# rezashkv/diffusion_pruning

Hardware: AMD Instinct MI355X
Metric: denoise-steps/s (SD-2.1 U-Net forward, 512x512, bs=4 per GPU, 50% channel mask) (higher is better)
Workload: dtype bf16

## Files before the change

### diffusion_pruning_amd/csrc/conv_gemm.hip

```cpp
#define APTP_CG_MAIN 1
#include "conv_gemm_core.h"

using namespace aptp_cg;

namespace {

template <typename T> struct Elem;
template <> struct Elem<__bf16> { static constexpr int EPC = 8, KS = 64; };
template <> struct Elem<float> { static constexpr int EPC = 4, KS = 32; };

template <int BM, int BN, int WM, int WN, typename T = __bf16>
__global__ __launch_bounds__(256) void conv_gemm_kernel(const KParams p) {
  static_assert(WM * WN == 4, "4 waves per workgroup");
  constexpr int EPC = Elem<T>::EPC, KS = Elem<T>::KS, ES = (int)sizeof(T);
  constexpr bool F32 = sizeof(T) == 4;
  constexpr int WTM = BM / WM, WTN = BN / WN;
  constexpr int MF = WTM / 16, NF = WTN / 16;
  constexpr int A_PASS = BM / 32, B_PASS = BN / 32;
  static_assert(BM % 32 == 0 && BN % 32 == 0 && WTM % 16 == 0 && WTN % 16 == 0, "tile shape");

  __shared__ __attribute__((aligned(16))) T smem[2 * (BM + BN) * KS];
  T* As = smem;
  T* Bs = smem + 2 * BM * KS;

// ... 1250 lines not shown
    mp = (M + kTiles[t].bm - 1) / kTiles[t].bm * kTiles[t].bm;
    np = ((int64_t)p->N + kTiles[t].bn - 1) / kTiles[t].bn * kTiles[t].bn;
  }
  return (int64_t)p->split_k * mp * np * (int64_t)sizeof(float);
}

extern "C" int aptp_conv_gemm_tiles(const AptpConvGemmParams* p) {
  if (!p) return 0;
  const int64_t M = (int64_t)p->B * p->Hout * p->Wout;
  const int t = pick_tile(p, (int)M);
  if (t <= 0 || t >= kNumTiles) return 0;
  return (int)(((M + kTiles[t].bm - 1) / kTiles[t].bm) * ((p->N + kTiles[t].bn - 1) / kTiles[t].bn));
}

extern "C" int aptp_conv_gemm_colstat_rows(const AptpConvGemmParams* p) {
  if (!p) return 0;
  const int t = pick_tile(p, p->B * p->Hout * p->Wout);
  if (t <= 0 || t >= kNumTiles) return 0;
  return kTiles[t].bm / (kTiles[t].nw / kTiles[t].wn);
}

extern "C" int aptp_conv_gemm_rowstat_slots(const AptpConvGemmParams* p) {
  if (!p) return 0;
  const int t = pick_tile(p, p->B * p->Hout * p->Wout);
  if (t <= 0 || t >= kNumTiles) return 0;
  return ((p->N + kTiles[t].bn - 1) / kTiles[t].bn) * kTiles[t].wn;
}

extern "C" int aptp_conv_gemm_suggest_split_k(const AptpConvGemmParams* p) {
  if (!p) return 1;
  const int M = p->B * p->Hout * p->Wout;
  const int t = pick_tile(p, M);
  const int64_t blocks = (int64_t)((M + kTiles[t].bm - 1) / kTiles[t].bm) * ((p->N + kTiles[t].bn - 1) / kTiles[t].bn);
  const int nK = p->KH * p->KW * (p->cin_pad / BK);
  if (blocks >= 256) return 1;
  int s = (int)((512 + blocks - 1) / blocks);
  const int max_s = nK / 8 > 0 ? nK / 8 : 1;
  if (s > max_s) s = max_s;
  if (s > 32) s = 32;
  return s < 1 ? 1 : s;
}

extern "C" int aptp_conv_gemm(const AptpConvGemmParams* p, aptp_stream_t stream) {
  KParams k;
  const int rc = fill_kparams(p, k);
  if (rc != APTP_OK) return rc;
  if (k.split_k > 1) APTP_CHECK(k.ws != nullptr && ((uintptr_t)k.ws % 16) == 0, "conv_gemm: split_k > 1 needs a 16B-aligned workspace");
  if (k.split_k == 1) k.counters = nullptr;
  k.gn_gamma = p->gn_gamma; k.gn_beta = p->gn_beta; k.gn_groups = p->gn_groups; k.gn_C = p->gn_C; k.gn_silu = p->gn_silu; k.gn_eps = p->gn_eps;
  if (k.gn_gamma) {
    APTP_CHECK(k.gn_beta && k.split_k > 1 && !k.counters && !k.out_f32 && k.act == APTP_ACT_NONE && !k.colgate && !k.corr && !k.residual && !k.depth
               && !k.rstat_out && !k.cstat_out && !k.ln_stats, "conv_gemm: gn_gamma needs a plain bf16 convolution split along K with a reduce launch");
    APTP_CHECK(k.gn_groups > 0 && k.gn_C > 0 && k.gn_C <= k.N && k.gn_C % k.gn_groups == 0 && k.gn_C % 8 == 0 && (k.gn_C / k.gn_groups) % 4 == 0
               && (int64_t)k.HW * (k.gn_C / k.gn_groups) <= 4LL * GN_RED_QPT * GN_RED_NT && k.ldy % 4 == 0,
               "conv_gemm: gn_gamma geometry (C=%d groups=%d HW=%d)", k.gn_C, k.gn_groups, k.HW);
  }
  hipStream_t s = (hipStream_t)stream;
  int t = pick_tile(p, k.M);
  if (t < 0 || t >= kNumTiles) { aptp_set_error("conv_gemm: unknown tile %d", t); return APTP_EINVAL; }
  if (k.io_f32 && t >= APTP_TILE_DMA_128x128) {
    aptp_set_error("conv_gemm: io_f32 (fp32 parity path) runs on the register-staged tiles 1..6 only (got tile %d)", t);
    return APTP_EINVAL;
  }
  if (t >= APTP_TILE_DMA_128x128 && !is_sk_tile(t) && (p->cin_pad * 2 > 8064 || (p->x2 && p->cin2_pad * 2 > 8064))) {
    aptp_set_error("conv_gemm: LDS-DMA tiles need Cin <= 4032 (got cin_pad %d)", p->cin_pad);
    return APTP_EINVAL;
  }
  if (k.rstat_out) {
    const int slots = ((k.N + kTiles[t].bn - 1) / kTiles[t].bn) * kTiles[t].wn;
    if ((k.split_k != 1 && !k.counters) || k.rstat_slots != slots) {
      aptp_set_error("conv_gemm: rowstat_out needs split_k == 1 (or the in-kernel reduction) and rowstat_slots == aptp_conv_gemm_rowstat_slots() (%d), got split_k %d, slots %d",
                     slots, k.split_k, k.rstat_slots);
      return APTP_EINVAL;
    }
  }
  if (k.cstat_out) {
    const int wtm = kTiles[t].bm / (kTiles[t].nw / kTiles[t].wn), wtn = kTiles[t].bn / kTiles[t].wn;
    if (!k.epi16 || k.act == APTP_ACT_GEGLU || (k.split_k != 1 && !k.counters) || k.HW % wtm != 0 || wtn < 32 ||
        k.cstat_ld < k.Nout || ((uintptr_t)k.cstat_out % 8) != 0) {
      aptp_set_error("conv_gemm: colstat_out needs the coalesced bf16 epilogue, no GEGLU, split_k == 1 (or the in-kernel reduction), "
                     "Hout*Wout %% %d == 0 (aptp_conv_gemm_colstat_rows) and colstat_ld >= N", wtm);
      return APTP_EINVAL;
    }
  }
  if (k.act == APTP_ACT_GEGLU && (kTiles[t].bn == 160)) {
    aptp_set_error("conv_gemm: GEGLU cannot use a 160-wide tile");
    return APTP_EINVAL;
  }
  {
    const int tiles_m = (k.M + kTiles[t].bm - 1) / kTiles[t].bm, tiles_n = (k.N + kTiles[t].bn - 1) / kTiles[t].bn;
    APTP_CHECK((int64_t)tiles_m * tiles_n * k.split_k < (1ll << 31) && (int64_t)k.nK * (k.split_k + 1) < (1ll << 31), "conv_gemm: grid too large");
    k.fd_hw = make_fastdiv(k.HW); k.fd_wout = make_fastdiv(k.Wout);
    k.fd_tm = make_fastdiv(tiles_m); k.fd_tn = make_fastdiv(tiles_n); k.fd_sk = make_fastdiv(k.split_k);
    k.fd_perm = make_fastdiv(tiles_n * k.split_k); k.fd_tmn = make_fastdiv(tiles_m * tiles_n);
  }
  static const bool lin_on = !(getenv("APTP_LIN") && getenv("APTP_LIN")[0] == '0');
  if (lin_on && p->epilogue != 2 && aptp_lin_eligible(k, t)) {
    const int rc2 = aptp_launch_lin(k, t, s);
    if (rc2 != APTP_OK) return rc2;
    APTP_LAUNCH_CHECK();
    return APTP_OK;
  }
  switch (t) {
    case APTP_TILE_128x128: launch_tile<128, 128>(k, s); break;
    case APTP_TILE_128x160: launch_tile<128, 160>(k, s); break;
    case APTP_TILE_64x128: launch_tile<64, 128>(k, s); break;
    case APTP_TILE_64x160: launch_tile<64, 160>(k, s); break;
    case APTP_TILE_128x64: launch_tile<128, 64>(k, s); break;
    case APTP_TILE_64x64: launch_tile<64, 64>(k, s); break;
    case APTP_TILE_DMA_128x128: launch_tile_dma<128, 128, 2>(k, s); break;
    case APTP_TILE_DMA_128x160: launch_tile_dma<128, 160, 2>(k, s); break;
    case APTP_TILE_DMA_64x128: launch_tile_dma<64, 128, 2>(k, s); break;
    case APTP_TILE_DMA_64x160: launch_tile_dma<64, 160, 2>(k, s); break;
    case APTP_TILE_DMA_128x64: launch_tile_dma<128, 64, 2>(k, s); break;
    case APTP_TILE_DMA_64x64: launch_tile_dma<64, 64, 2>(k, s); break;
    case APTP_TILE_DMA3_128x128: launch_tile_dma<128, 128, 3>(k, s); break;
    case APTP_TILE_DMA3_128x160: launch_tile_dma<128, 160, 3>(k, s); break;
    case APTP_TILE_DMA3_64x128: launch_tile_dma<64, 128, 3>(k, s); break;
    case APTP_TILE_DMA3_64x160: launch_tile_dma<64, 160, 3>(k, s); break;
    case APTP_TILE_DMA3_128x64: launch_tile_dma<128, 64, 3>(k, s); break;
    case APTP_TILE_DMA3_64x64: launch_tile_dma<64, 64, 3>(k, s); break;
    case APTP_TILE_DMA8_128x160: launch_tile_dma8<128, 160, 4, 2>(k, s); break;
    case APTP_TILE_DMA8_256x160: launch_tile_dma8<256, 160, 4, 2>(k, s); break;
    case APTP_TILE_DMA8_128x128: launch_tile_dma8<128, 128, 2, 4>(k, s); break;
    case APTP_TILE_DMA8_256x128: launch_tile_dma8<256, 128, 4, 2>(k, s); break;
    case APTP_TILE_DMA4_64x160: launch_tile_dma<64, 160, 4>(k, s); break;
    case APTP_TILE_DMA4_64x128: launch_tile_dma<64, 128, 4>(k, s); break;
    case APTP_TILE_DMA4_64x64: launch_tile_dma<64, 64, 4>(k, s); break;
    case APTP_TILE_DMA4_128x64: launch_tile_dma<128, 64, 4>(k, s); break;
    case APTP_TILE_DMA4_128x128: launch_tile_dma<128, 128, 4>(k, s); break;
    case APTP_TILE_DMA8R3_128x160: launch_tile_dma8<128, 160, 4, 2, 3>(k, s); break;
    case APTP_TILE_DMA8R4_128x160: launch_tile_dma8<128, 160, 4, 2, 4>(k, s); break;
    case APTP_TILE_DMA8R3_128x128: launch_tile_dma8<128, 128, 2, 4, 3>(k, s); break;
    case APTP_TILE_DMA8R4_128x128: launch_tile_dma8<128, 128, 2, 4, 4>(k, s); break;
    case APTP_TILE_DMA8R3_256x128: launch_tile_dma8<256, 128, 4, 2, 3>(k, s); break;
    case APTP_TILE_PP3_128x160: launch_tile_pp<128, 160, 4, 2, 3>(k, s); break;
    case APTP_TILE_PP4_128x160: launch_tile_pp<128, 160, 4, 2, 4>(k, s); break;
    case APTP_TILE_PP3_128x128: launch_tile_pp<128, 128, 2, 4, 3>(k, s); break;
    case APTP_TILE_PP4_128x128: launch_tile_pp<128, 128, 2, 4, 4>(k, s); break;
    case APTP_TILE_PP4_64x160: launch_tile_pp<64, 160, 4, 2, 4>(k, s); break;
    case APTP_TILE_PP4_64x128: launch_tile_pp<64, 128, 2, 4, 4>(k, s); break;
    case APTP_TILE_PP5_64x160: launch_tile_pp<64, 160, 4, 2, 5>(k, s); break;
    case APTP_TILE_PP4_128x64: launch_tile_pp<128, 64, 4, 2, 4>(k, s); break;
    case APTP_TILE_PP3_256x128: launch_tile_pp<256, 128, 4, 2, 3>(k, s); break;
    case APTP_TILE_PP3_128x256: launch_tile_pp<128, 256, 2, 4, 3>(k, s); break;
    case APTP_TILE_DMA6_64x64: launch_tile_dma<64, 64, 6>(k, s); break;
    case APTP_TILE_DMA8S_64x64: launch_tile_dma<64, 64, 8>(k, s); break;
    case APTP_TILE_DMA6_64x128: launch_tile_dma<64, 128, 6>(k, s); break;
    case APTP_TILE_DMA6_128x64: launch_tile_dma<128, 64, 6>(k, s); break;
    case APTP_TILE_KU2S4_64x64: launch_tile_ku2<64, 64, 2, 2, 4>(k, s); break;
    case APTP_TILE_KU2S6_64x64: launch_tile_ku2<64, 64, 2, 2, 6>(k, s); break;
    case APTP_TILE_KU2S4_64x128: launch_tile_ku2<64, 128, 2, 2, 4>(k, s); break;
    case APTP_TILE_KU2S6_64x128: launch_tile_ku2<64, 128, 2, 2, 6>(k, s); break;
    case APTP_TILE_KU2S4_128x64: launch_tile_ku2<128, 64, 2, 2, 4>(k, s); break;
    case APTP_TILE_KU2S4_128x128: launch_tile_ku2<128, 128, 2, 2, 4>(k, s); break;
    case APTP_TILE_KU2S4_64x160: launch_tile_ku2<64, 160, 2, 2, 4>(k, s); break;
    case APTP_TILE_KU2S4_128x160: launch_tile_ku2<128, 160, 4, 2, 4>(k, s); break;
    case APTP_TILE_KU2S4_128x128W8: launch_tile_ku2<128, 128, 2, 4, 4>(k, s); break;
    case APTP_TILE_KS2S3_64x64: launch_tile_ks2<64, 64, 3>(k, s); break;
    case APTP_TILE_KS2S4_64x64: launch_tile_ks2<64, 64, 4>(k, s); break;
    case APTP_TILE_KS2S3_64x128: launch_tile_ks2<64, 128, 3>(k, s); break;
    case APTP_TILE_KS2S4_64x128: launch_tile_ks2<64, 128, 4>(k, s); break;
    case APTP_TILE_KS2S3_128x64: launch_tile_ks2<128, 64, 3>(k, s); break;
    case APTP_TILE_KS2S3_128x128: launch_tile_ks2<128, 128, 3>(k, s); break;
    case APTP_TILE_SK_256x160: case APTP_TILE_SK_256x128: case APTP_TILE_SK_128x256:
    case APTP_TILE_SKL_256x160: case APTP_TILE_SKL_256x128: case APTP_TILE_SKL_128x256:
    case APTP_TILE_SK_128x160: case APTP_TILE_SKL_128x160: case APTP_TILE_SK_128x128: case APTP_TILE_SKL_128x128: {
      if (k.split_k > 1 && !k.counters) { aptp_set_error("conv_gemm: the stream-K tiles combine in-kernel: split_k > 1 needs tile_counters"); return APTP_EINVAL; }
      const int rc2 = aptp_launch_sk(k, t, s);
      if (rc2 != APTP_OK) return rc2;
      break;
    }
    case APTP_TILE_HALO_128x160:
    case APTP_TILE_HALO_128x128: {
      const int W = p->Wout;
      if (!(p->KH == 3 && p->KW == 3 && p->stride == 1 && p->pad == 1 && p->ups == 0 && !p->x2 && W > 0 && 128 % W == 0 &&
            (p->Hout * W) % 128 == 0 && (128 / W + 2) * (W + 2) <= 264)) {
        aptp_set_error("conv_gemm: the halo tiles need a 3x3 / stride-1 / pad-1 convolution without x2 whose width divides 128 (16, 32 or 64)");
        return APTP_EINVAL;
      }
      const int tiles = ((k.M + 127) / 128) * ((k.N + kTiles[t].bn - 1) / kTiles[t].bn);
      if (t == APTP_TILE_HALO_128x160) hipLaunchKernelGGL((conv3x3_halo_kernel<160, 4>), dim3(tiles * k.split_k), dim3(512), 0, s, k);
      else hipLaunchKernelGGL((conv3x3_halo_kernel<128, 4>), dim3(tiles * k.split_k), dim3(512), 0, s, k);
      break;
    }
// ... 16 lines not shown
```

### diffusion_pruning_amd/csrc/conv_gemm_core.h

```cpp
#pragma once
#include "aptp_common.h"
#if defined(APTP_STAMPS) && defined(APTP_CG_MAIN)
__device__ unsigned long long g_stamps[4096 * 4];
__device__ unsigned long long g_phase[4096 * 8];
#define APTP_PHASE(i) do { st_phase[i] = __builtin_readcyclecounter() - st_entry; } while (0)
__device__ unsigned long long g_epi[4096 * 8];
#define APTP_EPI(k) do { if ((threadIdx.x & 63) == 0) g_epi[((blockIdx.x * 8 + (threadIdx.x >> 6)) & 4095) * 8 + (k)] = __builtin_readcyclecounter(); } while (0)
#define APTP_STAMP(i) do { asm volatile("s_waitcnt lgkmcnt(0)" ::: "memory"); const unsigned long long t_ = __builtin_readcyclecounter(); \
    if ((i) > 0) st_acc[(i) - 1] += t_ - st_prev; st_prev = t_; } while (0)
#else
#define APTP_STAMP(i) do { } while (0)
#define APTP_PHASE(i) do { } while (0)
#define APTP_EPI(k) do { } while (0)
#endif
#ifndef APTP_ABLATE
#define APTP_ABLATE 0
#endif

namespace aptp_cg {


constexpr int BK = 64;
typedef __attribute__((ext_vector_type(4))) unsigned int u32x4;

// ... 273 lines not shown
    lna[i] += __shfl_xor(lna[i], 16); lna2[i] += __shfl_xor(lna2[i], 16);
    lna[i] += __shfl_xor(lna[i], 32); lna2[i] += __shfl_xor(lna2[i], 32);
    RowCtx rc;
    ln_finish(p, lna[i], lna2[i], rc);
    ln_mean[i] = rc.mean; ln_rstd[i] = rc.rstd;
  }
}

template <int MF, int NF, int WTM, int WTN, int WN>
__device__ __forceinline__ void tile_epilogue(const KParams& p, f32x4 (&acc)[MF][NF], int m0, int n0, int tn, int wm, int wn, int lane,
                                              const float (&ln_mean)[MF], const float (&ln_rstd)[MF]) {
  const int frow = lane & 15, fq = lane >> 4;
#pragma unroll
  for (int i = 0; i < MF; ++i) {
    const int m = m0 + wm * WTM + i * 16 + frow;
    if (m >= p.M) continue;
    RowCtx rc;
    row_info(p, m, rc);
    rc.mean = ln_mean[i]; rc.rstd = ln_rstd[i];
    float st[2] = {0.f, 0.f};
    if (p.act == APTP_ACT_GEGLU) {
      if constexpr (NF % 2 == 0) {
#pragma unroll
        for (int j = 0; j < NF; j += 2) {
          const int n = n0 + wn * WTN + j * 16 + fq * 4;
          if (n >= p.N) continue;
          float h[4] = {acc[i][j][0], acc[i][j][1], acc[i][j][2], acc[i][j][3]};
          float g[4] = {acc[i][j + 1][0], acc[i][j + 1][1], acc[i][j + 1][2], acc[i][j + 1][3]};
          epilogue_quad<true>(p, m, rc, n, h, g, st);
        }
      }
    } else {
#pragma unroll
      for (int j = 0; j < NF; ++j) {
        const int n = n0 + wn * WTN + j * 16 + fq * 4;
        if (n >= p.N) continue;
        float h[4] = {acc[i][j][0], acc[i][j][1], acc[i][j][2], acc[i][j][3]};
        epilogue_quad<false>(p, m, rc, n, h, h, st);
      }
    }
    if (p.rstat_out) {
      st[0] += __shfl_xor(st[0], 16); st[1] += __shfl_xor(st[1], 16);
      st[0] += __shfl_xor(st[0], 32); st[1] += __shfl_xor(st[1], 32);
      if (fq == 0) {
        float2 o; o.x = st[0]; o.y = st[1];
        const int slot = tn * WN + wn;
        reinterpret_cast<float2*>(p.rstat_out)[((int64_t)(slot >> 1) * p.M + m) * 2 + (slot & 1)] = o;
      }
    }
  }
}

constexpr float USTAT_SUM_SCALE = 1048576.0f;
constexpr float USTAT_SQ_SCALE = 4096.0f;
template <int WL>
__device__ __forceinline__ void emit_unit_stats(const KParams& p, const float (&tot)[2][(WL + 63) / 64], float* buf, int lane, int cw0,
                                                int row0) {
  __builtin_amdgcn_fence(__ATOMIC_ACQ_REL, "wavefront");
  __builtin_amdgcn_wave_barrier();
#pragma unroll
  for (int q = 0; q < (WL + 63) / 64; ++q) {
    const int t = lane + 64 * q;
    if (t < WL) { buf[t] = tot[0][q]; buf[WL + t] = tot[1][q]; }
  }
  __builtin_amdgcn_fence(__ATOMIC_ACQ_REL, "wavefront");
  __builtin_amdgcn_wave_barrier();
  const int cend = cw0 + WL < p.Nout ? cw0 + WL : p.Nout;
  if (cw0 >= cend || row0 >= p.M) return;
  const int unit = p.ustat_unit;
  const int u0 = cw0 / unit, u1 = (cend - 1) / unit;
  const int u = u0 + lane;
  if (u > u1) return;
  const int lo = (u * unit > cw0 ? u * unit : cw0) - cw0;
  const int hi = ((u + 1) * unit < cend ? (u + 1) * unit : cend) - cw0;
  float s = 0.f, s2 = 0.f;
  for (int c = lo; c < hi; ++c) { s += buf[c]; s2 += buf[WL + c]; }
  const int b = p.fd_hw.div(row0);
  const int rep = (int)blockIdx.x & (p.ustat_nrep - 1);
  unsigned long long* dst = reinterpret_cast<unsigned long long*>(p.ustat_out) + (((int64_t)rep * p.B + b) * p.ustat_units + u) * 2;
  __hip_atomic_fetch_add(dst, (unsigned long long)__float2ll_rn(s * USTAT_SUM_SCALE), __ATOMIC_RELAXED, __HIP_MEMORY_SCOPE_AGENT);
  __hip_atomic_fetch_add(dst + 1, (unsigned long long)__float2ll_rn(s2 * USTAT_SQ_SCALE), __ATOMIC_RELAXED, __HIP_MEMORY_SCOPE_AGENT);
}

template <bool GEGLU, int MF, int NF, int WTM, int WTN, int WN>
__device__ __forceinline__ void tile_epilogue_lds(const KParams& p, f32x4 (&acc)[MF][NF], int m0, int n0, int tn, int wm, int wn,
                                                  int lane, const float (&ln_mean)[MF], const float (&ln_rstd)[MF], float* buf) {
  constexpr int WL = GEGLU ? WTN / 2 : WTN;
  constexpr int PITCH = WL + 4;
  constexpr int LPR = WL / 8;
  constexpr int RPP = 64 / LPR;
  constexpr int NPASS = (16 + RPP - 1) / RPP;
  constexpr bool POW2 = (LPR & (LPR - 1)) == 0;
  const int frow = lane & 15, fq = lane >> 4;
  const int lrow = lane / LPR, lc8 = lane - lrow * LPR;
  const int c0 = (GEGLU ? ((n0 + wn * WTN) >> 1) : (n0 + wn * WTN)) + lc8 * 8;
  const bool lane_on = lrow < RPP && c0 < p.Nout;
  __bf16* const yb = reinterpret_cast<__bf16*>(p.y);
  float cs[8], cs2[8];
#pragma unroll
  for (int e = 0; e < 8; ++e) { cs[e] = 0.f; cs2[e] = 0.f; }
#pragma unroll
  for (int i = 0; i < MF; ++i) {
    const int mbase = m0 + wm * WTM + i * 16;
    u32x4 rres[NPASS], rdin[NPASS];
#pragma unroll
    for (int ps = 0; ps < NPASS; ++ps) {
      const int r = ps * RPP + lrow, m2 = mbase + r;
      const bool on = lane_on && r < 16 && m2 < p.M;
      rres[ps] = (u32x4){0u, 0u, 0u, 0u}; rdin[ps] = (u32x4){0u, 0u, 0u, 0u};
      if (on && p.residual && !(APTP_ABLATE & 64)) rres[ps] = *reinterpret_cast<const u32x4*>(p.residual + (int64_t)m2 * p.ldres + c0);
      if (on && p.depth && !(APTP_ABLATE & 64)) rdin[ps] = *reinterpret_cast<const u32x4*>(p.depth_in + (int64_t)m2 * p.lddin + c0);
    }
    {
      const int m = mbase + frow;
      RowCtx rc;
      row_info(p, m < p.M ? m : p.M - 1, rc);
      rc.mean = ln_mean[i]; rc.rstd = ln_rstd[i];
      if constexpr (GEGLU) {
        if constexpr (NF % 2 == 0) {
#pragma unroll
          for (int j = 0; j < NF; j += 2) {
            const int n = n0 + wn * WTN + j * 16 + fq * 4;
            float h[4] = {acc[i][j][0], acc[i][j][1], acc[i][j][2], acc[i][j][3]};
            float g[4] = {acc[i][j + 1][0], acc[i][j + 1][1], acc[i][j + 1][2], acc[i][j + 1][3]};
            float v[4] = {0.f, 0.f, 0.f, 0.f};
            if (n < p.N) {
              ColVecs cv;
              load_colvecs<true>(p, n, cv);
              epilogue_pre<true>(p, rc, n, cv, h, g, v);
            }
            *reinterpret_cast<float4*>(buf + frow * PITCH + (j / 2) * 16 + fq * 4) = make_float4(v[0], v[1], v[2], v[3]);
          }
        }
      } else {
#pragma unroll
        for (int j = 0; j < NF; ++j) {
          const int n = n0 + wn * WTN + j * 16 + fq * 4;
          float h[4] = {acc[i][j][0], acc[i][j][1], acc[i][j][2], acc[i][j][3]};
          float v[4] = {0.f, 0.f, 0.f, 0.f};
          if (n < p.N) {
            ColVecs cv;
            load_colvecs<false>(p, n, cv);
            epilogue_pre<false>(p, rc, n, cv, h, h, v);
          }
          *reinterpret_cast<float4*>(buf + frow * PITCH + j * 16 + fq * 4) = make_float4(v[0], v[1], v[2], v[3]);
        }
      }
    }
    __builtin_amdgcn_fence(__ATOMIC_ACQ_REL, "wavefront");
    __builtin_amdgcn_wave_barrier();
    if (i == 0) APTP_EPI(2);
#pragma unroll
    for (int ps = 0; ps < NPASS; ++ps) {
      const int r = ps * RPP + lrow, m2 = mbase + r;
      const bool on = lane_on && r < 16 && m2 < p.M;
      float v[8];
      {
        const int rr = r < 16 ? r : 15;
        const float4 a = *reinterpret_cast<const float4*>(buf + rr * PITCH + lc8 * 8);
        const float4 b4 = *reinterpret_cast<const float4*>(buf + rr * PITCH + lc8 * 8 + 4);
        v[0] = a.x; v[1] = a.y; v[2] = a.z; v[3] = a.w; v[4] = b4.x; v[5] = b4.y; v[6] = b4.z; v[7] = b4.w;
      }
      if (p.residual && !(APTP_ABLATE & 64)) {
        float f[8];
        union { u32x4 v; uint4 s; } cv; cv.v = rres[ps];
        unpack_bf16x8(cv.s, f);
#pragma unroll
        for (int e = 0; e < 8; ++e) v[e] += f[e];
      }
      if (p.depth && !(APTP_ABLATE & 64)) {
        const float d = p.depth[p.fd_hw.div(m2 < p.M ? m2 : p.M - 1) % p.depth_B];
        float f[8];
        union { u32x4 v; uint4 s; } cv; cv.v = rdin[ps];
        unpack_bf16x8(cv.s, f);
#pragma unroll
        for (int e = 0; e < 8; ++e) v[e] = (1.0f - d) * f[e] + d * v[e];
      }
      const uint4 o = pack_bf16x8(v);
#if APTP_ABLATE & 32
      asm volatile("" :: "v"(o.x), "v"(o.y), "v"(o.z), "v"(o.w));
#else
      if (on) *reinterpret_cast<uint4*>(yb + (int64_t)m2 * p.ldy + c0) = o;
#endif
      if constexpr (!GEGLU) {
        if (p.cstat_out && on) {
          float f[8];
          unpack_bf16x8(o, f);
#pragma unroll
          for (int e = 0; e < 8; ++e) { cs[e] += f[e]; cs2[e] += f[e] * f[e]; }
        }
      }
      if constexpr (POW2) {
        if (p.rstat_out) {
          float f[8], s0 = 0.f, s1 = 0.f;
          unpack_bf16x8(o, f);
          if (c0 < p.Nout) {
#pragma unroll
            for (int e = 0; e < 8; ++e) { s0 += f[e]; s1 += f[e] * f[e]; }
          }
#pragma unroll
          for (int off = 1; off < LPR; off <<= 1) { s0 += __shfl_xor(s0, off); s1 += __shfl_xor(s1, off); }
          if (lrow < RPP && r < 16 && m2 < p.M && lc8 == 0) {
            float2 q; q.x = s0; q.y = s1;
            const int slot = tn * WN + wn;
            reinterpret_cast<float2*>(p.rstat_out)[((int64_t)(slot >> 1) * p.M + m2) * 2 + (slot & 1)] = q;
          }
        }
      }
    }
    if (i == 0) APTP_EPI(3);
  }
  APTP_EPI(4);
  if constexpr (!GEGLU && WL >= 32) {
    if (p.cstat_out) {
      static_assert(RPP * WL <= 16 * PITCH, "column-statistics staging");
      float tot[2][(WL + 63) / 64];
#pragma unroll
      for (int ph = 0; ph < 2; ++ph) {
        if (lrow < RPP) {
          float* dst = buf + lrow * WL + lc8 * 8;
          if (ph == 0) {
            *reinterpret_cast<float4*>(dst) = make_float4(cs[0], cs[1], cs[2], cs[3]);
            *reinterpret_cast<float4*>(dst + 4) = make_float4(cs[4], cs[5], cs[6], cs[7]);
          } else {
            *reinterpret_cast<float4*>(dst) = make_float4(cs2[0], cs2[1], cs2[2], cs2[3]);
            *reinterpret_cast<float4*>(dst + 4) = make_float4(cs2[4], cs2[5], cs2[6], cs2[7]);
          }
        }
        __builtin_amdgcn_fence(__ATOMIC_ACQ_REL, "wavefront");
        __builtin_amdgcn_wave_barrier();
#pragma unroll
        for (int q = 0; q < (WL + 63) / 64; ++q) {
          const int t = lane + 64 * q;
          float a = 0.f;
          if (t < WL) {
#pragma unroll
            for (int r = 0; r < RPP; ++r) a += buf[r * WL + t];
          }
          tot[ph][q] = a;
        }
        __builtin_amdgcn_fence(__ATOMIC_ACQ_REL, "wavefront");
        __builtin_amdgcn_wave_barrier();
      }
      const int cw0 = n0 + wn * WTN;
      float2* dstg = reinterpret_cast<float2*>(p.cstat_out) + (int64_t)(m0 / WTM + wm) * p.cstat_ld;
#pragma unroll
      for (int q = 0; q < (WL + 63) / 64; ++q) {
        const int t = lane + 64 * q;
        if (t < WL && cw0 + t < p.Nout) dstg[cw0 + t] = make_float2(tot[0][q], tot[1][q]);
      }
      if (p.ustat_out) emit_unit_stats<WL>(p, tot, buf, lane, cw0, m0 + wm * WTM);
    }
  }
}

template <int NT, int MF, int NF>
__device__ __forceinline__ bool splitk_combine(const KParams& p, f32x4 (&acc)[MF][NF], int tile, int kz, int tid, int* lds_word) {
  constexpr int PER = MF * NF;
  float4* const slab = reinterpret_cast<float4*>(p.ws) + (int64_t)tile * p.split_k * (PER * NT);
  float4* const mine = slab + (int64_t)kz * (PER * NT);
  {
    const __amdgpu_buffer_rsrc_t srsrc = __builtin_amdgcn_make_buffer_rsrc(mine, 0, PER * NT * 16, 0x00020000);
#pragma unroll
    for (int i = 0; i < MF; ++i)
#pragma unroll
      for (int j = 0; j < NF; ++j) {
        __builtin_amdgcn_raw_buffer_store_b128(__builtin_bit_cast(u32x4, acc[i][j]), srsrc, ((i * NF + j) * NT + tid) * 16, 0, 16);
      }
  }
  asm volatile("s_waitcnt vmcnt(0)" ::: "memory");
  __syncthreads();
  if (tid == 0) *lds_word = __hip_atomic_fetch_add(p.counters + tile, 1, __ATOMIC_RELAXED, __HIP_MEMORY_SCOPE_AGENT);
  __syncthreads();
  const int ticket = *reinterpret_cast<volatile int*>(lds_word);
  if (ticket != p.split_k - 1) return false;
  if (tid == 0) {
    __hip_atomic_store(p.counters + tile, 0, __ATOMIC_RELAXED, __HIP_MEMORY_SCOPE_AGENT);
    __builtin_amdgcn_fence(__ATOMIC_ACQUIRE, "agent");
    asm volatile("s_waitcnt vmcnt(0)" ::: "memory");
  }
  __syncthreads();
#pragma unroll
  for (int i = 0; i < MF; ++i)
#pragma unroll
    for (int j = 0; j < NF; ++j) acc[i][j] = (f32x4){0.f, 0.f, 0.f, 0.f};
  for (int z = 0; z < p.split_k; ++z) {
    const float4* src = slab + (int64_t)z * (PER * NT);
    float4 t[MF][NF];
#pragma unroll
    for (int i = 0; i < MF; ++i)
#pragma unroll
      for (int j = 0; j < NF; ++j) t[i][j] = src[(i * NF + j) * NT + tid];
#pragma unroll
    for (int i = 0; i < MF; ++i)
#pragma unroll
      for (int j = 0; j < NF; ++j) {
        acc[i][j][0] += t[i][j].x; acc[i][j][1] += t[i][j].y; acc[i][j][2] += t[i][j].z; acc[i][j][3] += t[i][j].w;
      }
  }
  return true;
}

__device__ __forceinline__ void prefetch_next(const KParams& p, int tid, int nt, unsigned* scratch) {
  if (!p.pf_ptr) return;
  const int xcd = blockIdx.x & 7;
  aptp_prefetch_slice(p.pf_ptr, p.pf_bytes, xcd, blockIdx.x >> 3, ((int)gridDim.x + 7 - xcd) >> 3, tid, nt, scratch);
}

template <int NW, int MF, int NF, int WTM, int WTN, int WN>
__device__ __forceinline__ void run_epilogue(const KParams& p, f32x4 (&acc)[MF][NF], int m0, int n0, int tn, int wm, int wn, int lane,
                                             int wave, const float (&ln_mean)[MF], const float (&ln_rstd)[MF], __bf16* smem) {
  constexpr int PITCH_MAX = WTN + 4;
  constexpr bool POW2 = ((WTN / 8) & (WTN / 8 - 1)) == 0;
  if (p.epi16 && (POW2 || !p.rstat_out)) {
    APTP_EPI(0);
    __syncthreads();
    APTP_EPI(1);
    float* buf = reinterpret_cast<float*>(smem) + wave * 16 * PITCH_MAX;
    if (p.act == APTP_ACT_GEGLU) {
      if constexpr (NF % 2 == 0) tile_epilogue_lds<true, MF, NF, WTM, WTN, WN>(p, acc, m0, n0, tn, wm, wn, lane, ln_mean, ln_rstd, buf);
    } else {
      tile_epilogue_lds<false, MF, NF, WTM, WTN, WN>(p, acc, m0, n0, tn, wm, wn, lane, ln_mean, ln_rstd, buf);
    }
  } else {
    tile_epilogue<MF, NF, WTM, WTN, WN>(p, acc, m0, n0, tn, wm, wn, lane, ln_mean, ln_rstd);
  }
}

inline FastDiv make_fastdiv(int d) {
  FastDiv f;
  if (d <= 1) { f.mul = 0; f.shr = 0; f.one = ~0u; return f; }
  int l = 0;
  while ((1ll << l) < d) ++l;
  const int p = 31 + l;
  f.mul = (unsigned)(((1ull << p) + (unsigned)d - 1) / (unsigned)d);
  f.shr = (unsigned)(p - 32);
  f.one = 0;
  return f;
}

int aptp_sk_cus();
int aptp_launch_sk(const KParams& k, int tile, hipStream_t s);
bool aptp_lin_eligible(const KParams& k, int tile);
int aptp_launch_lin(const KParams& k, int tile, hipStream_t s);

}
```

Baseline: 203.8.

## Add lean 3x3 conv GEMM kernel with prefetched epilogue operands

Adds a specialized implicit-GEMM kernel for 3x3 convolutions with a simple epilogue (bias, row bias, gate, SiLU, correction, residual). It keeps per-row tap offset tables in registers and shifts them per tap instead of recomputing addresses. Bias, residual and correction operands are loaded before the K loop so their latency overlaps the main loop. The kernel is enabled by default for several tile configurations, and the column-stats code is factored into a shared helper. In exchange it adds register pressure and a separate code path to maintain.

```diff
diff --git a/diffusion_pruning_amd/csrc/conv_gemm.hip b/diffusion_pruning_amd/csrc/conv_gemm.hip
--- a/diffusion_pruning_amd/csrc/conv_gemm.hip
+++ b/diffusion_pruning_amd/csrc/conv_gemm.hip
@@ -1356,6 +1356,11 @@
                      "Hout*Wout %% %d == 0 (aptp_conv_gemm_colstat_rows) and colstat_ld >= N", wtm);
       return APTP_EINVAL;
     }
+    const int wl = k.act == APTP_ACT_GEGLU ? wtn / 2 : wtn;
+    if (k.ustat_out && (wl % k.ustat_unit == 0 ? wl / k.ustat_unit : (wl - 1) / k.ustat_unit + 2) > 64) {
+      aptp_set_error("conv_gemm: ustat_unit %d too small for the %d columns of a wave of tile %d (at most 64 units per wave)", k.ustat_unit, wl, t);
+      return APTP_EINVAL;
+    }
   }
   if (k.act == APTP_ACT_GEGLU && (kTiles[t].bn == 160)) {
     aptp_set_error("conv_gemm: GEGLU cannot use a 160-wide tile");
@@ -1375,6 +1380,11 @@
     APTP_LAUNCH_CHECK();
     return APTP_OK;
   }
+  static const bool lean_on = !(getenv("APTP_CONV_LEAN") && getenv("APTP_CONV_LEAN")[0] == '0');
+  if (lean_on && p->epilogue == 0 && aptp_conv_lean_eligible(k, t)) {
+    const int rc2 = aptp_launch_conv_lean(k, t, s);
+    if (rc2 != APTP_OK) return rc2;
+  } else
   switch (t) {
     case APTP_TILE_128x128: launch_tile<128, 128>(k, s); break;
     case APTP_TILE_128x160: launch_tile<128, 160>(k, s); break;
diff --git a/diffusion_pruning_amd/csrc/conv_gemm_core.h b/diffusion_pruning_amd/csrc/conv_gemm_core.h
--- a/diffusion_pruning_amd/csrc/conv_gemm_core.h
+++ b/diffusion_pruning_amd/csrc/conv_gemm_core.h
@@ -379,6 +379,46 @@
   __hip_atomic_fetch_add(dst + 1, (unsigned long long)__float2ll_rn(s2 * USTAT_SQ_SCALE), __ATOMIC_RELAXED, __HIP_MEMORY_SCOPE_AGENT);
 }
 
+template <int WL, int RPP>
+__device__ __forceinline__ void emit_col_stats(const KParams& p, const float (&cs)[8], const float (&cs2)[8], float* buf, int lane, int lrow,
+                                               int lc8, int cw0, int rblk, int row0) {
+  float tot[2][(WL + 63) / 64];
+#pragma unroll
+  for (int ph = 0; ph < 2; ++ph) {
+    if (lrow < RPP) {
+      float* dst = buf + lrow * WL + lc8 * 8;
+      if (ph == 0) {
+        *reinterpret_cast<float4*>(dst) = make_float4(cs[0], cs[1], cs[2], cs[3]);
+        *reinterpret_cast<float4*>(dst + 4) = make_float4(cs[4], cs[5], cs[6], cs[7]);
+      } else {
+        *reinterpret_cast<float4*>(dst) = make_float4(cs2[0], cs2[1], cs2[2], cs2[3]);
+        *reinterpret_cast<float4*>(dst + 4) = make_float4(cs2[4], cs2[5], cs2[6], cs2[7]);
+      }
+    }
+    __builtin_amdgcn_fence(__ATOMIC_ACQ_REL, "wavefront");
+    __builtin_amdgcn_wave_barrier();
+#pragma unroll
+    for (int q = 0; q < (WL + 63) / 64; ++q) {
+      const int t = lane + 64 * q;
+      float a = 0.f;
+      if (t < WL) {
+#pragma unroll
+        for (int r = 0; r < RPP; ++r) a += buf[r * WL + t];
+      }
+      tot[ph][q] = a;
+    }
+    __builtin_amdgcn_fence(__ATOMIC_ACQ_REL, "wavefront");
+    __builtin_amdgcn_wave_barrier();
+  }
+  float2* dstg = reinterpret_cast<float2*>(p.cstat_out) + (int64_t)rblk * p.cstat_ld;
+#pragma unroll
+  for (int q = 0; q < (WL + 63) / 64; ++q) {
+    const int t = lane + 64 * q;
+    if (t < WL && cw0 + t < p.Nout) dstg[cw0 + t] = make_float2(tot[0][q], tot[1][q]);
+  }
+  if (p.ustat_out) emit_unit_stats<WL>(p, tot, buf, lane, cw0, row0);
+}
+
 template <bool GEGLU, int MF, int NF, int WTM, int WTN, int WN>
 __device__ __forceinline__ void tile_epilogue_lds(const KParams& p, f32x4 (&acc)[MF][NF], int m0, int n0, int tn, int wm, int wn,
                                                   int lane, const float (&ln_mean)[MF], const float (&ln_rstd)[MF], float* buf) {
@@ -509,45 +549,161 @@
   }
   APTP_EPI(4);
   if constexpr (!GEGLU && WL >= 32) {
-    if (p.cstat_out) {
-      static_assert(RPP * WL <= 16 * PITCH, "column-statistics staging");
-      float tot[2][(WL + 63) / 64];
-#pragma unroll
-      for (int ph = 0; ph < 2; ++ph) {
-        if (lrow < RPP) {
-          float* dst = buf + lrow * WL + lc8 * 8;
-          if (ph == 0) {
-            *reinterpret_cast<float4*>(dst) = make_float4(cs[0], cs[1], cs[2], cs[3]);
-            *reinterpret_cast<float4*>(dst + 4) = make_float4(cs[4], cs[5], cs[6], cs[7]);
-          } else {
-            *reinterpret_cast<float4*>(dst) = make_float4(cs2[0], cs2[1], cs2[2], cs2[3]);
-            *reinterpret_cast<float4*>(dst + 4) = make_float4(cs2[4], cs2[5], cs2[6], cs2[7]);
-          }
-        }
-        __builtin_amdgcn_fence(__ATOMIC_ACQ_REL, "wavefront");
-        __builtin_amdgcn_wave_barrier();
-#pragma unroll
-        for (int q = 0; q < (WL + 63) / 64; ++q) {
-          const int t = lane + 64 * q;
-          float a = 0.f;
-          if (t < WL) {
-#pragma unroll
-            for (int r = 0; r < RPP; ++r) a += buf[r * WL + t];
-          }
-          tot[ph][q] = a;
-        }
-        __builtin_amdgcn_fence(__ATOMIC_ACQ_REL, "wavefront");
-        __builtin_amdgcn_wave_barrier();
-      }
-      const int cw0 = n0 + wn * WTN;
-      float2* dstg = reinterpret_cast<float2*>(p.cstat_out) + (int64_t)(m0 / WTM + wm) * p.cstat_ld;
-#pragma unroll
-      for (int q = 0; q < (WL + 63) / 64; ++q) {
-        const int t = lane + 64 * q;
-        if (t < WL && cw0 + t < p.Nout) dstg[cw0 + t] = make_float2(tot[0][q], tot[1][q]);
-      }
-      if (p.ustat_out) emit_unit_stats<WL>(p, tot, buf, lane, cw0, m0 + wm * WTM);
-    }
+    static_assert(RPP * WL <= 16 * PITCH, "column-statistics staging");
+    if (p.cstat_out) emit_col_stats<WL, RPP>(p, cs, cs2, buf, lane, lrow, lc8, n0 + wn * WTN, m0 / WTM + wm, m0 + wm * WTM);
+  }
+}
+
+template <int WTM, int WTN>
+struct LeanEpiIn {
+  static constexpr int LPR = WTN / 8, RPF = 64 / LPR, NPF = (16 + RPF - 1) / RPF, NP = (WTM / 16) * NPF;
+  float cb[8], rb[8], gm[8];
+  float cr[NP][8];
+  u32x4 res[NP];
+  bool one_b;
+};
+
+template <int WTM, int WTN>
+__device__ __forceinline__ void lean_epi_sample(const KParams& p, int b, int cc, float (&rb)[8], float (&gm)[8]) {
+  if (p.rowbias) {
+    const float4 a = *reinterpret_cast<const float4*>(p.rowbias + (int64_t)b * p.ld_rowbias + cc);
+    const float4 c = *reinterpret_cast<const float4*>(p.rowbias + (int64_t)b * p.ld_rowbias + cc + 4);
+    rb[0] = a.x; rb[1] = a.y; rb[2] = a.z; rb[3] = a.w; rb[4] = c.x; rb[5] = c.y; rb[6] = c.z; rb[7] = c.w;
+  }
+  if (p.colgate) {
+    const float* gr = p.colgate + (int64_t)(b % p.gate_B) * (p.N / p.gate_group);
+#pragma unroll
+    for (int e = 0; e < 8; ++e) gm[e] = gr[(cc + e) / p.gate_group];
+  }
+}
+
+template <int WTM, int WTN>
+__device__ __forceinline__ void lean_epi_load(const KParams& p, int m0, int n0, int wm, int wn, int lane, LeanEpiIn<WTM, WTN>& in) {
+  using E = LeanEpiIn<WTM, WTN>;
+  const int lrow = lane / E::LPR, lc8 = lane - lrow * E::LPR;
+  const int c0 = n0 + wn * WTN + lc8 * 8;
+  const int cc = c0 < p.Nout ? c0 : p.Nout - 8;
+  const int mw0 = m0 + wm * WTM;
+  const int mf = mw0 < p.M ? mw0 : p.M - 1, ml = mw0 + WTM - 1 < p.M ? mw0 + WTM - 1 : p.M - 1;
+  const int b0 = p.fd_hw.div(mf);
+  in.one_b = p.fd_hw.div(ml) == b0;
+#pragma unroll
+  for (int e = 0; e < 8; ++e) { in.cb[e] = 0.f; in.rb[e] = 0.f; in.gm[e] = 1.f; }
+  if (p.bias) {
+    const float4 a = *reinterpret_cast<const float4*>(p.bias + cc), c = *reinterpret_cast<const float4*>(p.bias + cc + 4);
+    in.cb[0] = a.x; in.cb[1] = a.y; in.cb[2] = a.z; in.cb[3] = a.w; in.cb[4] = c.x; in.cb[5] = c.y; in.cb[6] = c.z; in.cb[7] = c.w;
+  }
+  lean_epi_sample<WTM, WTN>(p, b0, cc, in.rb, in.gm);
+#pragma unroll
+  for (int q = 0; q < E::NP; ++q) {
+    const int i = q / E::NPF, ps = q - i * E::NPF;
+    const int r = ps * E::RPF + lrow, m2 = mw0 + i * 16 + (r < 16 ? r : 15);
+    const int mc = m2 < p.M ? m2 : p.M - 1;
+    in.res[q] = (u32x4){0u, 0u, 0u, 0u};
+    if (p.residual) in.res[q] = *reinterpret_cast<const u32x4*>(p.residual + (int64_t)mc * p.ldres + cc);
+#pragma unroll
+    for (int e = 0; e < 8; ++e) in.cr[q][e] = 0.f;
+    if (p.corr) {
+      RowCtx rc;
+      row_info(p, mc, rc);
+      const float* cp = p.corr + ((int64_t)(rc.b % p.corr_B) * 9 + rc.cls) * p.Nout + cc;
+      const float4 a = *reinterpret_cast<const float4*>(cp), c = *reinterpret_cast<const float4*>(cp + 4);
+      in.cr[q][0] = a.x; in.cr[q][1] = a.y; in.cr[q][2] = a.z; in.cr[q][3] = a.w;
+      in.cr[q][4] = c.x; in.cr[q][5] = c.y; in.cr[q][6] = c.z; in.cr[q][7] = c.w;
+    }
+  }
+}
+
+template <int MF, int NF, int WTM, int WTN>
+__device__ __forceinline__ void lean_epilogue(const KParams& p, f32x4 (&acc)[MF][NF], int m0, int n0, int wm, int wn, int lane,
+                                              const LeanEpiIn<WTM, WTN>& in, float* buf) {
+  using E = LeanEpiIn<WTM, WTN>;
+  constexpr int WL = WTN, PITCH = WL + 4, LPR = E::LPR, RPF = E::RPF, NPF = E::NPF;
+  static_assert(WL % 8 == 0 && WL >= 32 && RPF * WL <= 16 * PITCH, "transposed layout / column-statistics staging");
+  const int frow = lane & 15, fq = lane >> 4;
+  const int lrow = lane / LPR, lc8 = lane - lrow * LPR;
+  const int c0 = n0 + wn * WTN + lc8 * 8;
+  const int cc = c0 < p.Nout ? c0 : p.Nout - 8;
+  const bool lane_on = lrow < RPF && c0 < p.Nout;
+  const int mw0 = m0 + wm * WTM;
+  __bf16* const yb = reinterpret_cast<__bf16*>(p.y);
+  float cs[8], cs2[8];
+#pragma unroll
+  for (int e = 0; e < 8; ++e) { cs[e] = 0.f; cs2[e] = 0.f; }
+#pragma unroll
+  for (int i = 0; i < MF; ++i) {
+    if (i > 0) {
+      __builtin_amdgcn_fence(__ATOMIC_ACQ_REL, "wavefront");
+      __builtin_amdgcn_wave_barrier();
+    }
+#pragma unroll
+    for (int j = 0; j < NF; ++j) *reinterpret_cast<f32x4*>(buf + frow * PITCH + j * 16 + fq * 4) = acc[i][j];
+    __builtin_amdgcn_fence(__ATOMIC_ACQ_REL, "wavefront");
+    __builtin_amdgcn_wave_barrier();
+#pragma unroll
+    for (int ps = 0; ps < NPF; ++ps) {
+      const int q = i * NPF + ps;
+      const int r = ps * RPF + lrow, m2 = mw0 + i * 16 + r;
+      const bool on = lane_on && r < 16 && m2 < p.M;
+      float v[8];
+      {
+        const int rr = r < 16 ? r : 15;
+        const float4 a = *reinterpret_cast<const float4*>(buf + rr * PITCH + lc8 * 8);
+        const float4 b4 = *reinterpret_cast<const float4*>(buf + rr * PITCH + lc8 * 8 + 4);
+        v[0] = a.x; v[1] = a.y; v[2] = a.z; v[3] = a.w; v[4] = b4.x; v[5] = b4.y; v[6] = b4.z; v[7] = b4.w;
+      }
+      float rb[8], gm[8];
+#pragma unroll
+      for (int e = 0; e < 8; ++e) { rb[e] = in.rb[e]; gm[e] = in.gm[e]; }
+      if (!in.one_b && (p.rowbias || p.colgate)) {
+        const int mr = mw0 + i * 16 + (r < 16 ? r : 15), mc = mr < p.M ? mr : p.M - 1;
+        lean_epi_sample<WTM, WTN>(p, p.fd_hw.div(mc), cc, rb, gm);
+      }
+      if (p.bias) {
+#pragma unroll
+        for (int e = 0; e < 8; ++e) v[e] += in.cb[e];
+      }
+      if (p.rowbias) {
+#pragma unroll
+        for (int e = 0; e < 8; ++e) v[e] += rb[e];
+      }
+      if (p.colgate) {
+#pragma unroll
+        for (int e = 0; e < 8; ++e) v[e] *= gm[e];
+      }
+      if (p.act == APTP_ACT_SILU) {
+#pragma unroll
+        for (int e = 0; e < 8; ++e) v[e] = silu_f(v[e]);
+      }
+      if (p.corr) {
+#pragma unroll
+        for (int e = 0; e < 8; ++e) v[e] += in.cr[q][e];
+      }
+#if defined(__HIP_DEVICE_COMPILE__)
+#pragma unroll
+      for (int e = 0; e < 8; ++e) asm volatile("" : "+v"(v[e]));
+#endif
+      if (p.residual) {
+        float f[8];
+        union { u32x4 v; uint4 s; } cv; cv.v = in.res[q];
+        unpack_bf16x8(cv.s, f);
+#pragma unroll
+        for (int e = 0; e < 8; ++e) v[e] += f[e];
+      }
+      const uint4 o = pack_bf16x8(v);
+      if (on) *reinterpret_cast<uint4*>(yb + (int64_t)m2 * p.ldy + c0) = o;
+      if (p.cstat_out && on) {
+        float f[8];
+        unpack_bf16x8(o, f);
+#pragma unroll
+        for (int e = 0; e < 8; ++e) { cs[e] += f[e]; cs2[e] += f[e] * f[e]; }
+      }
+    }
+  }
+  if (p.cstat_out) {
+    __builtin_amdgcn_fence(__ATOMIC_ACQ_REL, "wavefront");
+    __builtin_amdgcn_wave_barrier();
+    emit_col_stats<WL, RPF>(p, cs, cs2, buf, lane, lrow, lc8, n0 + wn * WTN, m0 / WTM + wm, mw0);
   }
 }
 
@@ -640,5 +796,7 @@
 int aptp_launch_sk(const KParams& k, int tile, hipStream_t s);
 bool aptp_lin_eligible(const KParams& k, int tile);
 int aptp_launch_lin(const KParams& k, int tile, hipStream_t s);
-
-}
+bool aptp_conv_lean_eligible(const KParams& k, int tile);
+int aptp_launch_conv_lean(const KParams& k, int tile, hipStream_t s);
+
+}
diff --git a/diffusion_pruning_amd/csrc/conv_lean.hip b/diffusion_pruning_amd/csrc/conv_lean.hip
--- /dev/null
+++ b/diffusion_pruning_amd/csrc/conv_lean.hip
@@ -0,0 +1,312 @@
+#include "conv_gemm_core.h"
+
+namespace {
+using namespace aptp_cg;
+
+typedef __attribute__((address_space(3))) void* lds_ptr;
+typedef const __attribute__((address_space(1))) void* gbl_ptr;
+
+constexpr unsigned ZERO_OFF = 0x80000000u;
+constexpr int NTAB = 10;
+
+__device__ __forceinline__ void dma16(__amdgpu_buffer_rsrc_t r, __bf16* lds, unsigned voff, int soff) {
+#if defined(__HIP_DEVICE_COMPILE__)
+  __builtin_amdgcn_raw_ptr_buffer_load_lds(r, (lds_ptr)lds, 16, voff, soff, 0, 0);
+#endif
+}
+
+template <int BM, int BN, int WM, int WN, int STAGES, bool PP, int KU>
+__global__ __launch_bounds__(WM * WN * 64) void conv_lean_kernel(const KParams p) {
+  constexpr int NW = WM * WN, NT = NW * 64, RPP = NT / 8;
+  constexpr int WTM = BM / WM, WTN = BN / WN, MF = WTM / 16, NF = WTN / 16;
+  constexpr int A_PASS = BM / RPP, B_PASS = (BN + RPP - 1) / RPP;
+  constexpr int B_FULL = BN / RPP, NLD_LO = A_PASS + B_FULL, NLD_HI = A_PASS + B_PASS;
+  static_assert(NW == 4 || NW == 8, "4 or 8 waves");
+  static_assert(BM % RPP == 0 && WTM % 16 == 0 && WTN % 16 == 0 && BN % 8 == 0, "tile shape");
+  static_assert(NW * 16 * (WTN + 4) * 4 <= STAGES * (BM + BN) * BK * 2, "epilogue transpose buffer");
+
+  __shared__ __attribute__((aligned(16))) __bf16 smem[STAGES * (BM + BN) * BK];
+  __shared__ unsigned pf_scratch[64];
+  __bf16* As = smem;
+  __bf16* Bs = smem + STAGES * BM * BK;
+
+  const int tid = threadIdx.x, lane = tid & 63;
+  const int wave = __builtin_amdgcn_readfirstlane(tid >> 6);
+  const int wm = wave / WN, wn = wave % WN;
+  const int tiles_n = (p.N + BN - 1) / BN, tiles_m = (p.M + BM - 1) / BM;
+  int tm, tn, kz;
+  decode_block(p, tiles_m, tiles_n, tm, tn, kz);
+  const int m0 = tm * BM, n0 = tn * BN;
+  const int kt_begin = p.fd_sk.div(p.nK * kz);
+  const int kt_end = p.fd_sk.div(p.nK * (kz + 1));
+
+  if (p.pf_ptr) {
+    const int xcd = blockIdx.x & 7;
+    const int x0 = (int)(((int64_t)p.pf_lines * xcd) >> 3), x1 = (int)(((int64_t)p.pf_lines * (xcd + 1)) >> 3);
+    const int l0 = x0 + (int)(blockIdx.x >> 3) * p.pf_per;
+    const int l1 = l0 + p.pf_per < x1 ? l0 + p.pf_per : x1;
+    for (int l = l0 + tid; l < l1; l += NT)
+      __builtin_amdgcn_global_load_lds((gbl_ptr)(p.pf_ptr + (int64_t)l * 64), (lds_ptr)pf_scratch, 4, 0, 0);
+  }
+
+  const int rowbase = tid >> 3;
+  const unsigned schunk = (unsigned)((tid & 7) ^ ((rowbase >> 1) & 7));
+  unsigned tab[A_PASS][NTAB];
+#pragma unroll
+  for (int i = 0; i < A_PASS; ++i) {
+    const int m = m0 + rowbase + RPP * i;
+    if (m < p.M) {
+      const int b = p.fd_hw.div(m), rem = m - b * p.HW;
+      const int oy = p.fd_wout.div(rem), ox = rem - oy * p.Wout;
+      const int iy0 = oy * p.stride - 1, ix0 = ox * p.stride - 1, pix0 = b * p.Hin * p.Win;
+#pragma unroll
+      for (int t = 0; t < 9; ++t) {
+        int iy = iy0 + t / 3, ix = ix0 + t % 3;
+        const bool ok = (unsigned)iy < (unsigned)p.HinE && (unsigned)ix < (unsigned)p.WinE && !(p.zins & (iy | ix));
+        iy >>= p.ups; ix >>= p.ups;
+        tab[i][t] = ok ? ((unsigned)(pix0 + iy * p.Win + ix) * (unsigned)p.ldx) * 2u + schunk * 16u : ZERO_OFF;
+      }
+      tab[i][9] = p.x2 ? ((unsigned)m * (unsigned)p.ldx2) * 2u + schunk * 16u : ZERO_OFF;
+    } else {
+#pragma unroll
+      for (int t = 0; t < NTAB; ++t) tab[i][t] = ZERO_OFF;
+    }
+  }
+  unsigned boff[B_PASS];
+#pragma unroll
+  for (int i = 0; i < B_PASS; ++i) {
+    int n = n0 + rowbase + RPP * i;
+    n = n < p.N ? n : p.N - 1;
+    boff[i] = (unsigned)(n * (unsigned)p.Ktot) * 2u + schunk * 16u;
+  }
+  const bool tail_bad = (int)((p.ncc - 1) * BK + schunk * 8) >= p.Cin;
+  const bool tail_bad2 = (int)((p.ncc2 - 1) * BK + schunk * 8) >= p.Cin2;
+  const __amdgpu_buffer_rsrc_t xr = __builtin_amdgcn_make_buffer_rsrc(const_cast<__bf16*>(p.x), 0, p.x_bytes, 0x00020000);
+  const __amdgpu_buffer_rsrc_t x2r =
+      __builtin_amdgcn_make_buffer_rsrc(const_cast<__bf16*>(p.x2 ? p.x2 : p.x), 0, p.x2 ? p.x2_bytes : 0, 0x00020000);
+  const __amdgpu_buffer_rsrc_t wr = __builtin_amdgcn_make_buffer_rsrc(const_cast<__bf16*>(p.w), 0, p.w_bytes, 0x00020000);
+
+  int l_kt = kt_begin, l_tap = 0, l_cc = kt_begin;
+  if (kt_begin != 0) {
+    l_tap = kt_begin / p.ncc;
+    if (l_tap > 9) l_tap = 9;
+    l_cc = kt_begin - l_tap * p.ncc;
+  }
+  auto next_tap = [&]() {
+#pragma unroll
+    for (int i = 0; i < A_PASS; ++i)
+#pragma unroll
+      for (int t = 0; t + 1 < NTAB; ++t) tab[i][t] = tab[i][t + 1];
+  };
+  for (int t = 0; t < l_tap; ++t) next_tap();
+
+  auto issue_tile = [&](int stage) {
+    const bool seg2 = l_tap == 9;
+    const int ncur = seg2 ? p.ncc2 : p.ncc;
+    const bool pad = l_cc == ncur - 1 && (seg2 ? tail_bad2 : tail_bad);
+    const int sa = __builtin_amdgcn_readfirstlane(l_cc * (BK * 2));
+    const int sb = __builtin_amdgcn_readfirstlane(l_kt * (BK * 2));
+#pragma unroll
+    for (int i = 0; i < A_PASS; ++i) {
+      __bf16* dst = As + (stage * BM + wave * 8 + RPP * i) * BK;
+      if (seg2) dma16(x2r, dst, pad ? ZERO_OFF : tab[i][0], sa);
+      else dma16(xr, dst, pad ? ZERO_OFF : tab[i][0], sa);
+    }
+#pragma unroll
+    for (int i = 0; i < B_PASS; ++i) {
+      if (wave * 8 + RPP * i < BN) {
+        __bf16* dst = Bs + (stage * BN + wave * 8 + RPP * i) * BK;
+        dma16(wr, dst, boff[i], sb);
+      }
+    }
+    ++l_kt;
+    if (++l_cc == ncur) {
+      l_cc = 0;
+      if (l_tap < 9) {
+        ++l_tap;
+        next_tap();
+      }
+    }
+  };
+
+  f32x4 acc[MF][NF];
+#pragma unroll
+  for (int i = 0; i < MF; ++i)
+#pragma unroll
+    for (int j = 0; j < NF; ++j) acc[i][j] = (f32x4){0.f, 0.f, 0.f, 0.f};
+  const int frow = lane & 15, fq = lane >> 4;
+  auto compute = [&](int stage) {
+#pragma unroll
+    for (int s = 0; s < 2; ++s) {
+      bf16x8 af[MF], wf[NF];
+#pragma unroll
+      for (int i = 0; i < MF; ++i) {
+        const int r = wm * WTM + i * 16 + frow;
+        af[i] = *reinterpret_cast<const bf16x8*>(As + (stage * BM + r) * BK + ((s * 4 + fq) ^ ((r >> 1) & 7)) * 8);
+      }
+#pragma unroll
+      for (int j = 0; j < NF; ++j) {
+        const int r = wn * WTN + j * 16 + frow;
+        wf[j] = *reinterpret_cast<const bf16x8*>(Bs + (stage * BN + r) * BK + ((s * 4 + fq) ^ ((r >> 1) & 7)) * 8);
+      }
+#pragma unroll
+      for (int i = 0; i < MF; ++i)
+#pragma unroll
+        for (int j = 0; j < NF; ++j) acc[i][j] = __builtin_amdgcn_mfma_f32_16x16x32_bf16(wf[j], af[i], acc[i][j], 0, 0, 0);
+    }
+  };
+
+  constexpr int D = PP ? STAGES - 2 : (KU == 2 ? STAGES - 2 : STAGES - 1);
+  constexpr int DW = KU == 2 ? D - 2 : D - 1;
+  static_assert(STAGES >= 2 && D >= 1 && DW >= 0 && NLD_HI * DW <= 63, "ring");
+  static_assert(!PP || (NW == 8 && STAGES >= 3), "ping-pong: 8 waves, ring of >= 3 stages");
+  static_assert(KU == 1 || (!PP && STAGES >= 4 && STAGES % 2 == 0), "two K-tiles per barrier: pairs of stages");
+  const bool hi = (NLD_HI != NLD_LO) && (wave * 8 + RPP * (B_PASS - 1) < BN);
+  auto wait_ring = [&](bool full) {
+    if (full && DW > 0) {
+      if (hi) asm volatile("s_waitcnt vmcnt(%0)" ::"n"(NLD_HI * DW) : "memory");
+      else asm volatile("s_waitcnt vmcnt(%0)" ::"n"(NLD_LO * DW) : "memory");
+    } else {
+      asm volatile("s_waitcnt vmcnt(0)" ::: "memory");
+    }
+  };
+  const int n = kt_end - kt_begin;
+  const int pre = n < D ? n : D;
+  for (int t = 0; t < pre; ++t) issue_tile(t);
+  LeanEpiIn<WTM, WTN> ein;
+  if (p.split_k == 1) lean_epi_load<WTM, WTN>(p, m0, n0, wm, wn, lane, ein);
+
+  if (n > 0) {
+    wait_ring(pre == D);
+    __builtin_amdgcn_s_barrier();
+    asm volatile("" ::: "memory");
+    int cur_s = 0, nxt_s = D % STAGES;
+    if constexpr (PP) {
+      const int grp = wave >> 2;
+      if (grp == 1) {
+        __builtin_amdgcn_s_barrier();
+        asm volatile("" ::: "memory");
+      }
+      for (int kt = 0; kt < n; ++kt) {
+        const bool issue = kt + D < n;
+        if (issue) issue_tile(nxt_s);
+        __builtin_amdgcn_sched_barrier(0);
+        __builtin_amdgcn_s_barrier();
+        __builtin_amdgcn_sched_barrier(0);
+        asm volatile("" ::: "memory");
+        __builtin_amdgcn_s_setprio(1);
+        compute(cur_s);
+        __builtin_amdgcn_s_setprio(0);
+        asm volatile("" ::: "memory");
+        wait_ring(issue);
+        asm volatile("s_waitcnt lgkmcnt(0)" ::: "memory");
+        __builtin_amdgcn_sched_barrier(0);
+        __builtin_amdgcn_s_barrier();
+        __builtin_amdgcn_sched_barrier(0);
+        asm volatile("" ::: "memory");
+        cur_s = cur_s + 1 == STAGES ? 0 : cur_s + 1;
+        nxt_s = nxt_s + 1 == STAGES ? 0 : nxt_s + 1;
+      }
+      if (grp == 0) {
+        __builtin_amdgcn_s_barrier();
+        asm volatile("" ::: "memory");
+      }
+    } else if constexpr (KU == 2) {
+      for (int kt = 0; kt < n; kt += 2) {
+        const int ni = n - (kt + D);
+        if (ni >= 1) issue_tile(nxt_s);
+        if (ni >= 2) issue_tile(nxt_s + 1);
+        compute(cur_s);
+        if (kt + 1 < n) compute(cur_s + 1);
+        asm volatile("" ::: "memory");
+        wait_ring(ni >= 2);
+        asm volatile("s_waitcnt lgkmcnt(0)" ::: "memory");
+        __builtin_amdgcn_s_barrier();
+        asm volatile("" ::: "memory");
+        cur_s = cur_s + 2 == STAGES ? 0 : cur_s + 2;
+        nxt_s = nxt_s + 2 == STAGES ? 0 : nxt_s + 2;
+      }
+    } else {
+      for (int kt = 0; kt < n; ++kt) {
+        const bool issue = kt + D < n;
+        if (issue) issue_tile(nxt_s);
+        compute(cur_s);
+        asm volatile("" ::: "memory");
+        wait_ring(issue);
+        asm volatile("s_waitcnt lgkmcnt(0)" ::: "memory");
+        __builtin_amdgcn_s_barrier();
+        asm volatile("" ::: "memory");
+        cur_s = cur_s + 1 == STAGES ? 0 : cur_s + 1;
+        nxt_s = nxt_s + 1 == STAGES ? 0 : nxt_s + 1;
+      }
+    }
+  }
+
+  if (p.split_k > 1 && p.counters) {
+    if (!splitk_combine<NT, MF, NF>(p, acc, tm * tiles_n + tn, kz, tid, reinterpret_cast<int*>(smem))) return;
+    lean_epi_load<WTM, WTN>(p, m0, n0, wm, wn, lane, ein);
+  } else if (p.split_k > 1) {
+    float* ws = p.ws + (int64_t)kz * p.M * p.ws_ld;
+#pragma unroll
+    for (int i = 0; i < MF; ++i) {
+      const int m = m0 + wm * WTM + i * 16 + frow;
+      if (m >= p.M) continue;
+#pragma unroll
+      for (int j = 0; j < NF; ++j) {
+        const int nn = n0 + wn * WTN + j * 16 + fq * 4;
+        if (nn >= p.N) continue;
+        float4 o; o.x = acc[i][j][0]; o.y = acc[i][j][1]; o.z = acc[i][j][2]; o.w = acc[i][j][3];
+        *reinterpret_cast<float4*>(ws + (int64_t)m * p.ws_ld + nn) = o;
+      }
+    }
+    return;
+  }
+  __syncthreads();
+  lean_epilogue<MF, NF, WTM, WTN>(p, acc, m0, n0, wm, wn, lane, ein, reinterpret_cast<float*>(smem) + wave * 16 * (WTN + 4));
+}
+
+template <int BM, int BN, int WM, int WN, int STAGES, bool PP, int KU>
+void launch_lean(KParams k, hipStream_t s) {
+  const int grid = ((k.M + BM - 1) / BM) * ((k.N + BN - 1) / BN) * k.split_k;
+  k.pf_lines = 0; k.pf_per = 0;
+  if (k.pf_ptr) {
+    const int nper = (grid + 7) >> 3;
+    k.pf_lines = (int)(k.pf_bytes >> 6);
+    const int per_xcd = (k.pf_lines + 7) >> 3;
+    k.pf_per = (per_xcd + nper - 1) / nper;
+    if (k.pf_per < 1) k.pf_per = 1;
+  }
+  hipLaunchKernelGGL((conv_lean_kernel<BM, BN, WM, WN, STAGES, PP, KU>), dim3(grid), dim3(WM * WN * 64), 0, s, k);
+}
+
+}
+
+namespace aptp_cg {
+
+bool aptp_conv_lean_eligible(const KParams& k, int tile) {
+  if (k.KH != 3 || k.KW != 3 || k.pad != 1 || (k.stride != 1 && k.stride != 2)) return false;
+  if (k.io_f32 || k.out_f32 || !k.epi16 || k.ln_stats || k.rstat_out || k.depth) return false;
+  if (k.act != APTP_ACT_NONE && k.act != APTP_ACT_SILU) return false;
+  if (k.Nout < 8 || k.ncc < 1) return false;
+  switch (tile) {
+    case APTP_TILE_PP4_128x160: case APTP_TILE_PP4_128x64: case APTP_TILE_DMA8R3_128x160:
+    case APTP_TILE_DMA8R3_128x128: case APTP_TILE_DMA3_64x64: case APTP_TILE_KU2S4_128x160:
+      return true;
+    default: return false;
+  }
+}
+
+int aptp_launch_conv_lean(const KParams& k, int tile, hipStream_t s) {
+  switch (tile) {
+    case APTP_TILE_PP4_128x160: launch_lean<128, 160, 4, 2, 4, true, 1>(k, s); break;
+    case APTP_TILE_PP4_128x64: launch_lean<128, 64, 4, 2, 4, true, 1>(k, s); break;
+    case APTP_TILE_DMA8R3_128x160: launch_lean<128, 160, 4, 2, 3, false, 1>(k, s); break;
+    case APTP_TILE_DMA8R3_128x128: launch_lean<128, 128, 2, 4, 3, false, 1>(k, s); break;
+    case APTP_TILE_DMA3_64x64: launch_lean<64, 64, 2, 2, 3, false, 1>(k, s); break;
+    case APTP_TILE_KU2S4_128x160: launch_lean<128, 160, 4, 2, 4, false, 2>(k, s); break;
+    default: aptp_set_error("conv_lean: tile %d has no lean instantiation", tile); return APTP_EINVAL;
+  }
+  return APTP_OK;
+}
+
+}
```

Measured after the change: 208.1 (median of 6 runs). 2.1% higher.
